# irmakguzey/SPWGNN

Measured on AMD Instinct MI355X. Metric: towers/sec fwd+bwd, 6-block batch=65k, 1/2/4/8 MI355X; achieved HBM GB/s, higher is better.
Workload: dtype f32; 1 GPU; train step fwd+BCE+bwd+Adam, 6-block towers fully connected, 65536 towers/GPU, 5 MP steps, dropout 0.1, x6 math; towers_per_gpu=65536, global_batch=65536, n_global_nodes=393216, nodes_per_tower=6, nodes_per_gpu=393216, edges_per_gpu=1966080, mp_steps=5, math=x6, parallelism=dp1

## Files before the change

include/spwgnn.h:

```cpp
#ifndef SPWGNN_H
#define SPWGNN_H

#include <stddef.h>
#include <stdint.h>

#ifdef __cplusplus
extern "C" {
#endif

#define SPWGNN_ABI_VERSION 6

#define SPWGNN_OK 0
#define SPWGNN_E_ARG (-1)
#define SPWGNN_E_SHAPE (-2)
#define SPWGNN_E_RELATION (-3)
#define SPWGNN_E_WORKSPACE (-4)
#define SPWGNN_E_CAPACITY (-5)
#define SPWGNN_E_NOTRAIN (-6)

typedef void* spwgnn_stream_t;

typedef struct spwgnn_param_info {
    const char* name;
    int64_t offset;
    int32_t rows;
    int32_t cols;
} spwgnn_param_info;

int32_t spwgnn_version(void);
int32_t spwgnn_struct_size(int32_t which);
const char* spwgnn_strerror(int32_t status);
int32_t spwgnn_param_tensor_count(void);
int64_t spwgnn_param_count(void);
// ... 80 lines not shown
#define SPWGNN_MATH_F32 0
#define SPWGNN_MATH_X6 1
#define SPWGNN_MATH_BF16 2

#define SPWGNN_K_NONE 0
#define SPWGNN_K_EDGE_FWD 1
#define SPWGNN_K_NODE_FWD 2
#define SPWGNN_K_EDGE_BWD 3
#define SPWGNN_K_NODE_BWD 4
#define SPWGNN_K_ENC_EDGE 5
#define SPWGNN_K_ENC_EDGE_BWD 6
#define SPWGNN_K_WGRAD_W2 7
#define SPWGNN_K_DA 8
#define SPWGNN_K_WGRAD_WS 9
#define SPWGNN_K_ENC_NODE 10
#define SPWGNN_K_ENC_NODE_BWD 11

int64_t spwgnn_workspace_bytes(int32_t n_nodes, int32_t n_eblocks, int32_t mp_steps, int32_t training);

int32_t spwgnn_fused_path(const spwgnn_batch* batch, const spwgnn_run* run);

int32_t spwgnn_team_max_blocks(int32_t set);

int32_t spwgnn_forward(const float* params, const spwgnn_batch* batch, const spwgnn_run* run,
                       void* workspace, int64_t workspace_bytes, float* logits,
                       spwgnn_stream_t stream);

int32_t spwgnn_backward(const float* params, const spwgnn_batch* batch, const spwgnn_run* run,
                        void* workspace, int64_t workspace_bytes, const float* dlogits,
                        float* grads, float* dprop, spwgnn_stream_t stream);

int64_t spwgnn_bce_scratch_bytes(int64_t n);
int32_t spwgnn_bce(const float* logits, const float* targets, int64_t n, float* out3,
                   float* dlogits, void* scratch, spwgnn_stream_t stream);
int32_t spwgnn_bce_accumulate(const float* logits, const float* targets, int64_t n, float* out3,
                              float* dlogits, void* scratch, const double* weights3, double* total3,
                              spwgnn_stream_t stream);
int32_t spwgnn_bce_backward(const float* params, const spwgnn_batch* batch, const spwgnn_run* run,
                            void* workspace, int64_t workspace_bytes, const float* logits,
                            const float* targets, int64_t n, float* out3, float* dlogits, void* bce_scratch,
                            const double* weights3, double* total3, float* grads, float* dprop,
                            spwgnn_stream_t stream);

int32_t spwgnn_adam(float* params, const float* grads, float* m, float* v, int64_t n, int32_t step,
                    float lr, float beta1, float beta2, float eps, float l2, float grad_scale,
                    spwgnn_stream_t stream);
// ... 31 lines not shown
```

spwgnn_amd/_lib.py:

```python
from __future__ import annotations

import ctypes as C
import os
from pathlib import Path
from typing import Optional

_LIB_PATH = Path(__file__).resolve().parent / "libspwgnn_hip.so"
_lib: Optional[C.CDLL] = None


class SpwgnnError(RuntimeError):
    pass


class ParamInfo(C.Structure):
    _fields_ = [("name", C.c_char_p), ("offset", C.c_int64), ("rows", C.c_int32), ("cols", C.c_int32)]


class PlanSizes(C.Structure):
    _fields_ = [("n_wtiles", C.c_int32), ("n_eblocks", C.c_int32), ("nw_max", C.c_int32)]


class BatchC(C.Structure):
    _fields_ = [
# ... 1 lines not shown
        ("nw_max", C.c_int32), ("flags", C.c_int32),
        ("pos", C.c_void_p), ("prop", C.c_void_p), ("node_tower", C.c_void_p), ("node_local", C.c_void_p),
        ("wtile", C.c_void_p), ("edge_src", C.c_void_p), ("edge_dst", C.c_void_p), ("blk_csr", C.c_void_p),
    ]


class PrologueC(C.Structure):
    _fields_ = [("copy_src", C.c_void_p), ("copy_dst", C.c_void_p), ("copy_bytes", C.c_int64),
                ("key", C.c_void_p), ("step", C.c_void_p), ("mode", C.c_int32), ("rank", C.c_int32),
                ("seed", C.c_uint64)]


class RunC(C.Structure):
    _fields_ = [("mp_steps", C.c_int32), ("training", C.c_int32), ("dropout", C.c_float), ("math", C.c_int32),
                ("seed", C.c_uint64), ("prof_kernel", C.c_int32), ("prof_count", C.c_int32),
                ("prof_events", C.c_void_p), ("seed_dev", C.c_void_p), ("prologue", C.c_void_p),
                ("grads_early_event", C.c_void_p)]


K_EDGE_FWD, K_NODE_FWD, K_EDGE_BWD, K_NODE_BWD, K_ENC_EDGE, K_ENC_EDGE_BWD, K_WGRAD_W2, K_DA = 1, 2, 3, 4, 5, 6, 7, 8
K_WGRAD_WS, K_ENC_NODE, K_ENC_NODE_BWD = 9, 10, 11
MATH_F32, MATH_X6, MATH_BF16 = 0, 1, 2
STEP_KEY_COUNTER, STEP_KEY_SPLITMIX = 0, 1
ABI_VERSION = 6
BATCH_RECV_BLOCKS = 1
READOUT_SUM_PROB, READOUT_MEAN_PROB, READOUT_SUM_LOGIT, READOUT_MEAN_LOGIT = 0, 1, 2, 3


def _declare(lib: C.CDLL) -> None:
    i32, i64, vp, f32 = C.c_int32, C.c_int64, C.c_void_p, C.c_float
    sig = {
        "spwgnn_version": (i32, []),
        "spwgnn_struct_size": (i32, [i32]),
        "spwgnn_strerror": (C.c_char_p, [i32]),
        "spwgnn_param_tensor_count": (i32, []),
        "spwgnn_param_count": (i64, []),
        "spwgnn_param_real_count": (i64, []),
        "spwgnn_param_tensor": (i32, [i32, C.POINTER(ParamInfo)]),
        "spwgnn_dense_to_edges": (i32, [vp, vp, i32, i32, vp, vp, vp, i64, C.POINTER(i64), vp]),
        "spwgnn_plan_size": (i32, [i32, vp, vp, i32, C.POINTER(PlanSizes)]),
        "spwgnn_plan_fill": (i32, [i32, vp, vp, vp, vp, i32, C.POINTER(PlanSizes), vp, vp, vp, vp, vp]),
        "spwgnn_plan_size_cap": (i32, [i32, vp, vp, i32, C.POINTER(PlanSizes)]),
        "spwgnn_plan_order": (i32, [i32, vp, vp, i32, vp]),
        "spwgnn_plan_fill_cap": (i32, [i32, vp, vp, vp, vp, vp, i32, C.POINTER(PlanSizes), vp, vp, vp, vp, vp]),
        "spwgnn_plan_size_recv": (i32, [i32, vp, i32, C.POINTER(PlanSizes)]),
        "spwgnn_plan_fill_recv": (i32, [i32, vp, vp, vp, vp, i32, C.POINTER(PlanSizes), vp, vp, vp, vp, vp]),
        "spwgnn_workspace_bytes": (i64, [i32, i32, i32, i32]),
        "spwgnn_fused_path": (i32, [C.POINTER(BatchC), C.POINTER(RunC)]),
        "spwgnn_team_max_blocks": (i32, [i32]),
        "spwgnn_host_device_ptr": (i32, [vp, C.POINTER(vp)]),
        "spwgnn_forward": (i32, [vp, C.POINTER(BatchC), C.POINTER(RunC), vp, i64, vp, vp]),
        "spwgnn_backward": (i32, [vp, C.POINTER(BatchC), C.POINTER(RunC), vp, i64, vp, vp, vp, vp]),
        "spwgnn_bce_scratch_bytes": (i64, [i64]),
        "spwgnn_bce": (i32, [vp, vp, i64, vp, vp, vp, vp]),
        "spwgnn_bce_accumulate": (i32, [vp, vp, i64, vp, vp, vp, vp, vp, vp]),
        "spwgnn_bce_backward": (i32, [vp, vp, vp, vp, i64, vp, vp, i64, vp, vp, vp, vp, vp, vp, vp, vp]),
        "spwgnn_adam": (i32, [vp, vp, vp, vp, i64, i32, f32, f32, f32, f32, f32, f32, vp]),
        "spwgnn_adam_dev": (i32, [vp, vp, vp, vp, i64, vp, vp, i32, f32, f32, f32, f32, f32, vp]),
        "spwgnn_adam_lr_table": (i32, [f32, f32, f32, i32, vp]),
        "spwgnn_step_advance": (i32, [vp, vp, i32, C.c_uint64, i32, vp]),
        "spwgnn_sigmoid": (i32, [vp, vp, i64, vp]),
        "spwgnn_copy_in": (i32, [vp, vp, i64, vp]),
        "spwgnn_accumulate_out3": (i32, [vp, vp, vp, vp]),
        "spwgnn_tower_readout": (i32, [vp, vp, i32, i32, vp, vp]),
    }
    for name, (res, args) in sig.items():
        fn = getattr(lib, name)
        fn.restype = res
        fn.argtypes = args


def lib() -> C.CDLL:
# ... 55 lines not shown
```

spwgnn_amd/csrc/api.hip:

```cpp
#include <cmath>
#include <cstring>
#include <cstdlib>
#include "kernels.h"
#include <vector>
#include "../../include/spwgnn.h"
static_assert(SPWGNN_MATH_F32 == spw::MATH_F32 && SPWGNN_MATH_X6 == spw::MATH_X6 && SPWGNN_MATH_BF16 == spw::MATH_BF16,
              "math ids");

namespace spw {

static inline int64_t up(int64_t x, int64_t a) { return (x + a - 1) / a * a; }

struct Ws {
    int64_t total = 0;
    int S, training;
    int64_t RN, RE, NB;
    int64_t pk;
    int64_t cw;
    int64_t zo1, co, P, a, o1, U, V, H2s;
    int64_t A, z1, z2, z3, cr;
    int64_t ed;
    int64_t mask1, mask2, zmask;
    int64_t dx, do1, g, G3, dU, dV, dP, dco, dzo2, dzo1;
    int64_t dA, dz4, dz3, dz2, dz1;
// ... 228 lines not shown
    hipStream_t st;
    mutable int k = 0;
    hipError_t before(int kid) const {
        if (r->prof_kernel != kid || !r->prof_events || k >= r->prof_count) return hipSuccess;
        return hipEventRecord(static_cast<hipEvent_t>(r->prof_events[2 * k]), st);
    }
    hipError_t after(int kid) const {
        if (r->prof_kernel != kid || !r->prof_events || k >= r->prof_count) return hipSuccess;
        hipError_t e = hipEventRecord(static_cast<hipEvent_t>(r->prof_events[2 * k + 1]), st);
        ++k;
        return e;
    }
};

#define SPW_CHECK(x)                                  \
    do {                                              \
        hipError_t e_ = (x);                          \
        if (e_ != hipSuccess) return (int32_t)e_;     \
    } while (0)

static bool rebuild_dA(const spwgnn_run* r, const spwgnn_batch* b) {
    const int m = kmath(r, kX6EdgeBwd);
    return b->nw_max <= 16 && m != MATH_F32 && !(m == MATH_X6 && !team_blocks(b->n_wtiles) && getenv_flag("SPWGNN_DA_RMW"));
}

static bool store_b16(const spwgnn_run* r, const spwgnn_batch* b) {
    return r->training && r->math == MATH_BF16 && kmath(r, kX6EncEdge) == MATH_BF16 &&
           kmath(r, kX6EncEdgeBwd) == MATH_BF16 && kmath(r, kX6Wgrad) == MATH_BF16 && rebuild_dA(r, b) &&
           !getenv_flag("SPWGNN_WG_OLD");
}

static bool store_b16_node(const spwgnn_run* r, const spwgnn_batch* b) {
    return store_b16(r, b) && kmath(r, kX6EdgeFwd) == MATH_BF16 && kmath(r, kX6NodeFwd) == MATH_BF16 &&
           kmath(r, kX6NodeBwd) == MATH_BF16 && kmath(r, kX6EdgeBwd) == MATH_BF16 && b->nw_max <= 16 &&
           !team_blocks(b->n_wtiles) && !team_blocks((b->n_nodes + 31) / 32) && !getenv_flag("SPWGNN_NODE_F32");
}

static int uv_storage(const spwgnn_run* r, const spwgnn_batch* b) {
    if (!r->training || r->math != MATH_BF16) return kUvF32;
    return store_b16_node(r, b) ? kUvB16 : kUvRound;
}

static bool fwd_fused_taken(const spwgnn_run* r, const spwgnn_batch* b) {
    const bool one_math = r->math == kmath(r, kX6EncEdge) && r->math == kmath(r, kX6EdgeFwd) &&
                          r->math == kmath(r, kX6NodeFwd);
    return one_math && fwd_fused_team(b->n_wtiles, b->nw_max, b->n_eblocks, b->n_nodes, r->math) &&
// ... 426 lines not shown
    if (!wsb || n < 2 || first < 0 || first + n > wsb->n || getenv_flag("SPWGNN_WS_NOGROUP")) return;
    const WsJob& j0 = wsb->j[first];
    const int w0 = (first + 1 < wsb->n ? wsb->j[first + 1].wg0 : wsb->wgs) - j0.wg0;
    if (w0 <= 0 || w0 % 8) return;
    for (int i = 1; i < n; ++i) {
        const WsJob& ji = wsb->j[first + i];
        const int wi = (first + i + 1 < wsb->n ? wsb->j[first + i + 1].wg0 : wsb->wgs) - ji.wg0;
        if (wi != w0 || ji.a.stages_per_wg != j0.a.stages_per_wg || ji.a.nbs != j0.a.nbs || ji.a.S != j0.a.S) return;
    }
    for (int i = 0; i < n; ++i) {
        wsb->j[first + i].gn = n;
        wsb->j[first + i].gi = i;
    }
}

int32_t run_backward(const float* params, const spwgnn_batch* b, const spwgnn_run* r, const Ws& w, char* base,
                     const float* dlogits, float* grads, float* dprop, hipStream_t st, const BceArgs* bce = nullptr) {
    (void)params;
    Ctx c{w, base};
    const int S = r->mp_steps;
    const bool rebuild = rebuild_dA(r, b);
    const bool b16 = store_b16(r, b);
    const bool n16 = store_b16_node(r, b);
    const int64_t nN = b->n_nodes;
    const float scale = (r->dropout > 0.f) ? 1.0f / (1.0f - r->dropout) : 1.0f;
    const bool zero_prop = b->prop == nullptr, need_dP0 = dprop != nullptr;
    const bool ws_skip0 = zero_prop && kmath(r, kX6Wgrad) != MATH_F32 && !getenv_flag("SPWGNN_WG_OLD");
    const bool skip_eb0 = rebuild && ws_skip0 && !need_dP0 && !team_blocks(b->n_wtiles);
    Prof prof{r, st};

    auto node_args = [&](int s) {
        const bool first = (s == S - 1);
        NodeBwdArgs nb{};
        nb.n_nodes = b->n_nodes;
        nb.first = first;
        nb.tail = 0;
        nb.dPin = first ? nullptr : c.f(w.dP_at(s + 1));
        nb.dU = first ? nullptr : c.f(w.dU_at(s + 1));
        nb.dV = first ? nullptr : c.f(w.dV_at(s + 1));
        nb.Pn = c.f(w.P_at(s + 1));
        nb.o1 = c.f(w.o1_at(s));
        nb.a = c.f(w.a_at(s));
        nb.dlogits = dlogits;
        nb.dx = c.f(w.dx_at(s));
        nb.do1 = c.f(w.do1_at(s));
        nb.g = c.f(w.g_at(s));
// ... 29 lines not shown
        return nb;
    };
    auto edge_args = [&](int s) {
        EdgeBwdArgs eb{};
        eb.n_wtiles = b->n_wtiles;
        eb.nw_max = b->nw_max;
        eb.wpg = b->nw_max <= 16 ? 4 : edge_wpg(edge_bwd_lds_per_wave(b->nw_max));
        eb.dA_accumulate = s != S - 1;
        eb.no_dA = rebuild;
        eb.wtile = b->wtile;
        eb.esrc = b->edge_src;
        eb.edst = b->edge_dst;
        eb.csr = reinterpret_cast<const uint32_t*>(b->blk_csr);
        eb.mask1 = c.u(w.m1_at(s));
        eb.mask2 = c.u(w.m2_at(s));
        eb.dh2_out = nullptr;
        eb.G3 = c.f(w.G3_at(s));
        eb.w2t = c.pk(PK_W2T);
        eb.x_w2t = r->math != MATH_F32 ? c.x6(X6_W2T) : nullptr;
        eb.dA = c.f(w.dA);
        eb.dU = c.f(w.dU_at(s));
        eb.dV = c.f(w.dV_at(s));
        eb.n16 = n16;
        return eb;
    };
    NodeBwdArgs tl{};
    if (dprop) {
        tl.n_nodes = b->n_nodes;
        tl.first = 0;
        tl.tail = 1;
        tl.dPin = c.f(w.dP_at(0));
        tl.dU = c.f(w.dU_at(0));
        tl.dV = c.f(w.dV_at(0));
        tl.dprop = dprop;
        tl.w1bt = c.pk(PK_W1BT);
        tl.w1ct = c.pk(PK_W1CT);
        if (r->math != MATH_F32) {
            tl.x_w1bt = c.x6(X6_W1BT);
            tl.x_w1ct = c.x6(X6_W1CT);
            tl.xh_w1bt = c.x6(X6_W1BT_H);
            tl.xh_w1ct = c.x6(X6_W1CT_H);
        }
        tl.n16 = n16;
    }
    DaArgs da{};
    if (rebuild) {
        da.n_eblocks = b->n_eblocks;
        da.S = S;
        da.g3_step = w.G3_at(1) - w.G3_at(0);
        da.m1_step = w.m1_at(1) - w.m1_at(0);
        da.m2_step = w.m2_at(1) - w.m2_at(0);
        da.edst = b->edge_dst;
        da.mask1 = c.u(w.mask1);
        da.mask2 = c.u(w.mask2);
        da.G3 = c.f(w.G3);
        da.dA = c.f(w.dA);
        da.x_w2t = c.x6(X6_W2T);
        da.b16 = b16;
    }
    EncEdgeBwdArgs eeb{};
    eeb.n_eblocks = b->n_eblocks;
    eeb.b16 = b16;
    eeb.dA = c.f(w.dA);
    eeb.zmask = c.u(w.zmask);
    eeb.w1at = c.pk(PK_W1AT);
    eeb.rm3t = c.pk(PK_RM3T);
    eeb.rm2t = c.pk(PK_RM2T);
    eeb.rm1t = c.pk(PK_RM1T);
    if (r->math != MATH_F32) {
        eeb.x_w1at = c.x6(X6_W1AT);
        eeb.x_rm3t = c.x6(X6_RM3T);
        eeb.x_rm2t = c.x6(X6_RM2T);
        eeb.x_rm1t = c.x6(X6_RM1T);
    }
    eeb.dz4 = c.f(w.dz4);
    eeb.dz3 = c.f(w.dz3);
    eeb.dz2 = c.f(w.dz2);
    eeb.dz1 = c.f(w.dz1);
    eeb.scale = scale;
    EncNodeBwdArgs enb{};
    enb.n_nodes = b->n_nodes;
// ... 309 lines not shown
int32_t spwgnn_fused_path(const spwgnn_batch* batch, const spwgnn_run* run) {
    const int32_t stt = validate(batch, run);
    if (stt) return stt;
    return (fwd_fused_taken(run, batch) ? 1 : 0) | (run->training && bwd_fused_taken(run, batch) ? 2 : 0);
}

int32_t spwgnn_host_device_ptr(const void* host, void** dev) {
    if (!host || !dev) return SPWGNN_E_ARG;
    void* p = nullptr;
    const hipError_t e = hipHostGetDevicePointer(&p, const_cast<void*>(host), 0);
    if (e != hipSuccess) {
        (void)hipGetLastError();
        return (int32_t)e;
    }
    if (!p) return SPWGNN_E_ARG;
    *dev = p;
    return SPWGNN_OK;
}

int32_t spwgnn_team_max_blocks(int32_t set) {
    return team_max_blocks(set);
}

int32_t spwgnn_forward(const float* params, const spwgnn_batch* batch, const spwgnn_run* run, void* workspace,
                       int64_t workspace_bytes, float* logits, spwgnn_stream_t stream) {
    int32_t stt = validate(batch, run);
    if (stt) return stt;
    if (!params || !workspace || !logits) return SPWGNN_E_ARG;
    Ws w = make_ws(batch->n_nodes, batch->n_eblocks, run->mp_steps, run->training ? 1 : 0);
    if (workspace_bytes < w.total) return SPWGNN_E_WORKSPACE;
    return run_forward(params, batch, run, w, static_cast<char*>(workspace), logits,
                       static_cast<hipStream_t>(stream));
}

int32_t spwgnn_backward(const float* params, const spwgnn_batch* batch, const spwgnn_run* run, void* workspace,
                        int64_t workspace_bytes, const float* dlogits, float* grads, float* dprop,
                        spwgnn_stream_t stream) {
    int32_t stt = validate(batch, run);
    if (stt) return stt;
    if (!run->training) return SPWGNN_E_NOTRAIN;
    if (!params || !workspace || !dlogits || !grads) return SPWGNN_E_ARG;
    Ws w = make_ws(batch->n_nodes, batch->n_eblocks, run->mp_steps, 1);
    if (workspace_bytes < w.total) return SPWGNN_E_WORKSPACE;
    return run_backward(params, batch, run, w, static_cast<char*>(workspace), dlogits, grads, dprop,
                        static_cast<hipStream_t>(stream));
}
// ... 152 lines not shown
```

spwgnn_amd/csrc/kernels.h:

```cpp
#pragma once

#ifndef SPWGNN_ONEHOT_BPERM
#define SPWGNN_ONEHOT_BPERM 1
#endif
#include "gemm_blocks.h"

namespace spw {

struct PackDesc {
    int64_t dst_off;
    int64_t src_off;
    int32_t rows, cols;
    int32_t src_rows, src_cols;
    int32_t src_ld, src_row0;
    int32_t transpose, perm;
    int32_t k4;
    int32_t bias_row;
    int64_t bias_off;
};
struct PrologueArgs {
    const uint4* src;
    uint4* dst;
    int64_t n16;
    uint64_t* key;
// ... 142 lines not shown
    int dco_sum;
    const float *w1bt, *w1ct, *wo2t, *wo1ct, *wo1at, *wo1pt, *w3t;
    const uint4 *x_w1bt, *x_w1ct, *x_wo2t, *x_wo1ct, *x_wo1at, *x_wo1pt, *x_w3t;
    const uint4 *xh_w1bt, *xh_w1ct, *xh_wo2t, *xh_wo1ct, *xh_wo1at, *xh_wo1pt;
    int n16;
    const float *bce_logits, *bce_targets;
    float* bce_dlogits;
    int64_t bce_n;
    int no_dP;
};

struct EdgeBwdArgs {
    int n_wtiles, nw_max, wpg;
    int dA_accumulate;
    int no_dA;
    const int32_t *wtile, *esrc, *edst;
    const uint32_t* csr;
    const uint32_t *mask1, *mask2;
    const float *G3, *w2t;
    float *dA, *dU, *dV;
    float* dh2_out;
    const uint4* x_w2t;
    int n16;
};

struct DaArgs {
    int n_eblocks, S;
    int b16;
    int64_t g3_step, m1_step, m2_step;
    const int32_t* edst;
    const uint32_t *mask1, *mask2;
    const float* G3;
    float* dA;
    const uint4* x_w2t;
};

struct EncEdgeBwdArgs {
    int n_eblocks;
    int b16;
    const float* dA;
    const uint32_t* zmask;
    const float *w1at, *rm3t, *rm2t, *rm1t;
    const uint4 *x_w1at, *x_rm3t, *x_rm2t, *x_rm1t;
    float *dz4, *dz3, *dz2, *dz1;
    float scale;
};

struct EncNodeBwdArgs {
    int n_nodes;
    float* dco;
    const float *co, *zo1, *om1t;
    const float* pos;
    const float *w_om0, *b_om0;
    const float* wo1ct;
    const float* do1;
    int64_t do1_step;
    int S;
// ... 146 lines not shown
    float* slab;
    int64_t nblk, blk_per_wg, count;
};
struct Pos3Batch {
    Pos3Args e, n;
    int ce, cn;
    int b16e;
};
hipError_t launch_wgrad_pos3(const Pos3Batch& p, hipStream_t st);
hipError_t launch_bce(const BceArgs& a, hipStream_t st);
hipError_t launch_adam(const AdamArgs& a, hipStream_t st);
hipError_t launch_step_advance(uint64_t* key, int32_t* step, int mode, uint64_t seed, int32_t rank, hipStream_t st);
hipError_t launch_sigmoid(const float* z, float* p, int64_t n, hipStream_t st);
hipError_t launch_accumulate_out3(const float* out3, const double* w, double* tot, hipStream_t st);
hipError_t launch_copy_in(const void* src, void* dst, int64_t n16, hipStream_t st);
hipError_t launch_tower_readout(const float* z, const int32_t* off, int n_towers, int mode, float* out, hipStream_t st);

#ifndef SPWGNN_TEAM_MAX_BLOCKS
#define SPWGNN_TEAM_MAX_BLOCKS 512
#endif
constexpr int kTeamMaxBlocks = SPWGNN_TEAM_MAX_BLOCKS;
bool team_blocks(int n_blocks);
int team_max_blocks(int set);
hipError_t launch_enc_node_team(const EncNodeArgs& a, int math, hipStream_t st);
hipError_t launch_edge_fwd_team(const EdgeFwdArgs& a, int math, hipStream_t st);
hipError_t launch_edge_bwd_team(const EdgeBwdArgs& a, int math, hipStream_t st);
hipError_t launch_dA_team(const DaArgs& a, int math, hipStream_t st);
hipError_t launch_enc_node_bwd_team(const EncNodeBwdArgs& a, int math, hipStream_t st);
hipError_t launch_node_fwd_team(const NodeFwdArgs& a, int math, hipStream_t st);
hipError_t launch_node_bwd_team(const NodeBwdArgs& a, int math, hipStream_t st);
hipError_t launch_enc_edge_team(const EncEdgeArgs& a, int math, bool train, hipStream_t st);
bool enc_pair_team(int n_eblocks, int n_nodes, int math);
hipError_t launch_enc_pair_team(const EncEdgeArgs& e, const EncNodeArgs& n, int math, bool train, hipStream_t st);
hipError_t launch_enc_edge_bwd_team(const EncEdgeBwdArgs& a, int math, hipStream_t st);
struct FwdFusedArgs {
    EncEdgeArgs ee;
    EncNodeArgs en;
    EdgeFwdArgs ef;
    NodeFwdArgs nf;
    int S, training;
    int encoders;
    int64_t rowsN, rowsE;
    int64_t m1_step, m2_step;
    float* logits;
};
bool fwd_fused_team(int n_wtiles, int nw_max, int n_eblocks, int n_nodes, int math);
// ... 27 lines not shown
```

spwgnn_amd/csrc/kernels_bwd.hip:

```cpp
#include "kernels.h"
#include <cstdlib>

namespace spw {

__global__ __launch_bounds__(256, 2) __attribute__((amdgpu_waves_per_eu(2, 2))) void k_node_bwd(NodeBwdArgs a) {
    const int lane = threadIdx.x & 63, h = lane >> 5, j = lane & 31;
    const int nb = blockIdx.x * 4 + (threadIdx.x >> 6);
    if (nb * 32 >= a.n_nodes) return;
    const int n = nb * 32 + j;
    const bool valid = n < a.n_nodes;
    const int64_t bN = (int64_t)nb * kCmBlkN, bE = (int64_t)nb * kCmBlk;
    const int pj = (h * 32 + j) * 4;

    f32x16 D[4];
    if (a.first) {
        zero_tiles(D);
    } else {
        load_cm<4>(a.dPin + bN, D, lane);
        tgemm_stream_acc<4, kKhE, kLdN, 64>(a.dU + bE + pj, D, a.w1bt, lane);
        tgemm_stream_acc<4, kKhE, kLdN, 64>(a.dV + bE + pj, D, a.w1ct, lane);
    }
    if (a.tail) {
        if (valid) {
#pragma unroll
// ... 635 lines not shown
    return hipGetLastError();
}
#ifndef SPWGNN_EBWD_PF
#define SPWGNN_EBWD_PF 2
#endif
#ifndef SPWGNN_EBWD_PF_B16
#define SPWGNN_EBWD_PF_B16 5
#endif
#ifndef SPWGNN_DA_PF_B16
#define SPWGNN_DA_PF_B16 5
#endif
#ifndef SPWGNN_DA_INTERLEAVE
#define SPWGNN_DA_INTERLEAVE 1
#endif
#ifndef SPWGNN_DA_LOCKSTEP
#define SPWGNN_DA_LOCKSTEP 1
#endif
#ifndef SPWGNN_OH_KB
#define SPWGNN_OH_KB 5
#endif
#ifndef SPWGNN_DA_DBG
#define SPWGNN_DA_DBG 0
#endif
template <bool ACCUM, bool NODA = false, int NP = 3, int DBG = 0, bool N16 = false>
__global__ __launch_bounds__(512, 1) __attribute__((amdgpu_waves_per_eu(2, 2))) void k_edge_bwd_x6(EdgeBwdArgs a) {
    constexpr int PF = NP == 1 ? SPWGNN_EBWD_PF_B16 : SPWGNN_EBWD_PF, kWaves = 8;
    __shared__ uint4 wl[50 * 3 * 64];
    for (int idx = threadIdx.x; idx < 50 * 3 * 64; idx += blockDim.x) wl[idx] = a.x_w2t[idx];
    __syncthreads();
    const int lane = threadIdx.x & 63, h = lane >> 5, i = lane & 31;
    const int wave = __builtin_amdgcn_readfirstlane(threadIdx.x >> 6);
    const int4* wtiles = reinterpret_cast<const int4*>(a.wtile);
    const int wstep = gridDim.x * kWaves;
    const WlBases wlb(wl + lane);
    struct Pre { int d, s; uint32_t w[5]; };
    auto load_pre = [&](int blk) {
        Pre p;
        const int64_t e = (int64_t)blk * 32 + i;
        p.d = a.edst[e];
        p.s = a.esrc[e];
        load_m2(a.mask2 + (int64_t)blk * kM2Blk, i, p.w);
        return p;
    };
    auto g_of = [&](int d, int n0) {
        return reinterpret_cast<const float4*>(a.G3 + cm_index<kKhE>(DBG == 3 ? n0 : (d >= 0 ? d : n0), 0) + h * 128);
    };
    struct KB { float4 g[2]; };
    auto ld = [&](const float4* G4, int kb, KB& r) {
// ... 85 lines not shown
            }
            bf16x8 ap[3];
            ap[0] = as_bf16x8(make_uint4(hw[0], hw[1], hw[2], hw[3]));
            ap[1] = as_bf16x8(make_uint4(mw[0], mw[1], mw[2], mw[3]));
            ap[2] = as_bf16x8(make_uint4(lw[0], lw[1], lw[2], lw[3]));
#pragma unroll
            for (int T = 0; T < 5; ++T) {
                const int u = (kb * 5 + T) * 3 * 64;
                bf16x8 bp[3];
                bp[0] = as_bf16x8(wlb.at(u));
                bp[1] = as_bf16x8(wlb.at(u + 64));
                bp[2] = as_bf16x8(wlb.at(u + 128));
                acc[T] = mfma32_x6<NP>(ap, bp, acc[T]);
            }
            __builtin_amdgcn_sched_barrier(0);
        }
#pragma unroll
        for (int t = 0; t < 5; ++t) {
            const uint32_t mh = m1w[t] >> (4 * h);
#pragma unroll
            for (int r = 0; r < 16; ++r) acc[t][r] = mask_bit(acc[t][r], mh, rho(r, 0));
        }
        float* dArow = a.dA + (int64_t)blk * 32 * kLdE + i;
#if SPWGNN_ONEHOT_BPERM && SPWGNN_OH_KB >= 10
        build_oh();
#endif
#pragma unroll
        for (int s = 0; s < 2; ++s) {
            uint32_t oh[4];
#pragma unroll
            for (int m = 0; m < 4; ++m) {
#if SPWGNN_ONEHOT_BPERM
                oh[m] = oh2[s][m];
#else
                uint32_t wv = 0u;
#pragma unroll
                for (int q = 0; q < 2; ++q) {
                    const int e = 2 * m + q;
                    const int d0 = __builtin_amdgcn_readlane(d, rho(8 * s + e, 0));
                    const int d1 = __builtin_amdgcn_readlane(d, rho(8 * s + e, 1));
                    const int s0 = __builtin_amdgcn_readlane(s_, rho(8 * s + e, 0));
                    const int s1 = __builtin_amdgcn_readlane(s_, rho(8 * s + e, 1));
                    const int node = i < 16 ? (h ? d1 : d0) : (h ? s1 : s0);
                    wv |= (node == key ? 0x3F80u : 0u) << (16 * q);
                }
                oh[m] = wv;
#endif
            }
            const bf16x8 ao = as_bf16x8(make_uint4(oh[0], oh[1], oh[2], oh[3]));
#pragma unroll
            for (int t = 0; t < 5; ++t) {
                uint32_t hw[4], mw[4], lw[4];
#pragma unroll
                for (int m = 0; m < 4; ++m) split2(acc[t][8 * s + 2 * m], acc[t][8 * s + 2 * m + 1], hw[m], mw[m], lw[m]);
                if constexpr (NP == 3) {
                    nacc[t] = __builtin_amdgcn_mfma_f32_32x32x16_bf16(ao, as_bf16x8(make_uint4(lw[0], lw[1], lw[2], lw[3])), nacc[t], 0, 0, 0);
                    nacc[t] = __builtin_amdgcn_mfma_f32_32x32x16_bf16(ao, as_bf16x8(make_uint4(mw[0], mw[1], mw[2], mw[3])), nacc[t], 0, 0, 0);
                }
                nacc[t] = __builtin_amdgcn_mfma_f32_32x32x16_bf16(ao, as_bf16x8(make_uint4(hw[0], hw[1], hw[2], hw[3])), nacc[t], 0, 0, 0);
#pragma unroll
                for (int r = 8 * s; r < 8 * s + 8; ++r) {
                    float* p = dArow + rho(r, h) * kLdE + 32 * t;
                    if constexpr (NODA) {
                    } else if (ACCUM) *p += acc[t][r];
                    else *p = acc[t][r];
                }
            }
        }
        cur = nxt;
        G4 = NG4;
    }
#pragma unroll
    for (int r = 0; r < 16; ++r) {
        const int row = rho(r, h);
        const int node = row & 15;
        if (node < nn) {
            float* o = row < 16 ? a.dV : a.dU;
#pragma unroll
            for (int t = 0; t < 5; ++t)
                if (32 * t + i < 2 * kKhE) {
                    if constexpr (N16) store_b16(o, cm_index<kKhE>(n0 + node, 32 * t + i), nacc[t][r]);
                    else o[cm_index<kKhE>(n0 + node, 32 * t + i)] = nacc[t][r];
                }
        }
    }
    info = ninfo;
    }
}

hipError_t launch_edge_bwd(const EdgeBwdArgs& a, int math, hipStream_t st) {
    if (math != MATH_F32 && a.nw_max <= 16 && a.no_dA && team_blocks(a.n_wtiles))
        return a.n16 ? hipErrorInvalidValue : launch_edge_bwd_team(a, math, st);
    if (a.n16 && (math != MATH_BF16 || a.nw_max > 16 || !a.no_dA)) return hipErrorInvalidValue;
    if (math != MATH_F32 && a.nw_max <= 16) {
        const dim3 g(edge_grid(a.n_wtiles, 8)), b(512);
        if (a.no_dA) {
#ifdef SPWGNN_DIAG
            static const int edbg = getenv("SPWGNN_EBWD_DBG") ? atoi(getenv("SPWGNN_EBWD_DBG")) : 0;
            if (math == MATH_BF16 && edbg == 3) {
                hipLaunchKernelGGL((k_edge_bwd_x6<false, true, 1, 3>), g, b, 0, st, a);
                return hipGetLastError();
            }
#endif
            if (math == MATH_BF16 && a.n16) hipLaunchKernelGGL((k_edge_bwd_x6<false, true, 1, 0, true>), g, b, 0, st, a);
            else if (math == MATH_BF16) hipLaunchKernelGGL((k_edge_bwd_x6<false, true, 1>), g, b, 0, st, a);
            else hipLaunchKernelGGL((k_edge_bwd_x6<false, true>), g, b, 0, st, a);
            return hipGetLastError();
        }
#ifdef SPWGNN_DIAG
        if (math != MATH_X6) return hipErrorInvalidValue;
        if (a.dA_accumulate) hipLaunchKernelGGL((k_edge_bwd_x6<true>), g, b, 0, st, a);
        else hipLaunchKernelGGL((k_edge_bwd_x6<false>), g, b, 0, st, a);
        return hipGetLastError();
#else
        return hipErrorInvalidValue;
#endif
    }
    if (a.nw_max <= 16) {
        if (a.dA_accumulate)
            hipLaunchKernelGGL((k_edge_bwd<true, true>), dim3(edge_grid(a.n_wtiles)), dim3(64 * kEdgeWaves), 0, st, a);
        else
            hipLaunchKernelGGL((k_edge_bwd<true, false>), dim3(edge_grid(a.n_wtiles)), dim3(64 * kEdgeWaves), 0, st, a);
    } else {
        const size_t lds = edge_bwd_lds_per_wave(a.nw_max) * a.wpg;
        const dim3 g((a.n_wtiles + a.wpg - 1) / a.wpg), b(64 * a.wpg);
        if (math == MATH_BF16) {
            if (a.dA_accumulate) hipLaunchKernelGGL((k_edge_bwd<false, true, true>), g, b, lds, st, a);
            else hipLaunchKernelGGL((k_edge_bwd<false, false, true>), g, b, lds, st, a);
        } else if (a.dA_accumulate) {
            hipLaunchKernelGGL((k_edge_bwd<false, true>), g, b, lds, st, a);
        } else {
            hipLaunchKernelGGL((k_edge_bwd<false, false>), g, b, lds, st, a);
        }
    }
    return hipGetLastError();
}

template <int NP = 3, bool B16 = false>
__global__ __launch_bounds__(512, 1) __attribute__((amdgpu_waves_per_eu(2, 2))) void k_dA_x6(DaArgs a) {
    constexpr int kWaves = 8, PF = NP == 1 ? SPWGNN_DA_PF_B16 : 2;
    static_assert(10 % PF == 0, "ring slots carry over between (block, step) pairs");
    __shared__ uint4 wl[50 * 3 * 64];
    for (int idx = threadIdx.x; idx < 50 * 3 * 64; idx += blockDim.x) wl[idx] = a.x_w2t[idx];
    __syncthreads();
    const int lane = threadIdx.x & 63, h = lane >> 5, i = lane & 31;
    const int wave = __builtin_amdgcn_readfirstlane(threadIdx.x >> 6);
    const WlBases wlb(wl + lane);
#if SPWGNN_DA_INTERLEAVE
    constexpr int kStride = kWaves;
    const int perw = ((a.n_eblocks + gridDim.x - 1) / gridDim.x + kWaves - 1) / kWaves * kWaves;
    const int b0 = blockIdx.x * perw + wave, b1 = min(blockIdx.x * perw + perw, a.n_eblocks);
    const int wg_b0 = blockIdx.x * perw;
    const int rounds = SPWGNN_DA_LOCKSTEP ? max(0, (b1 - wg_b0 + kWaves - 1) / kWaves) : 0;
    const int mine = SPWGNN_DA_LOCKSTEP ? max(0, (b1 - b0 + kWaves - 1) / kWaves) : 0;
#else
    constexpr int kStride = 1;
    const int nw = gridDim.x * kWaves, gw = blockIdx.x * kWaves + wave;
    const int per = (a.n_eblocks + nw - 1) / nw;
    const int b0 = gw * per, b1 = min(b0 + per, a.n_eblocks);
#endif
#if SPWGNN_DA_INTERLEAVE && SPWGNN_DA_LOCKSTEP
    auto tail_barriers = [&](int done) {
// ... 10 lines not shown
    auto load_pair = [&](int blk, int s, int d) {
        Pair p;
        const bool valid = d >= 0;
        p.G4 = reinterpret_cast<const float4*>(a.G3 + s * a.g3_step + cm_index<kKhE>(valid && SPWGNN_DA_DBG == 0 ? d : 0, 0) + h * 128);
        const uint32_t* m1 = a.mask1 + s * a.m1_step + (int64_t)blk * kLdE + i;
        if (SPWGNN_DA_DBG >= 2) {
#pragma unroll
            for (int t = 0; t < 5; ++t) p.w[t] = p.m1w[t] = valid ? 0x5a5a5a5au ^ (uint32_t)(blk * 5 + t) : 0u;
            return p;
        }
        load_m2(a.mask2 + s * a.m2_step + (int64_t)blk * kM2Blk, i, p.w);
#pragma unroll
        for (int t = 0; t < 5; ++t) {
            p.w[t] = valid ? p.w[t] : 0u;
            p.m1w[t] = m1[32 * t];
        }
        return p;
    };
    struct KB { float4 g[2]; };
    auto ld = [&](const float4* G4, int kb, KB& r) {
#pragma unroll
        for (int c = 0; c < 2; ++c) r.g[c] = G4[64 * min(2 * kb + c, kKhE / 4 - 1)];
    };
    int blk = b0, s = a.S - 1;
    int d = a.edst[(int64_t)blk * 32 + i];
    Pair cur = load_pair(blk, s, d);
    KB ring[PF];
#pragma unroll
    for (int k = 0; k < PF; ++k) ld(cur.G4, k, ring[k]);
    f32x16 dacc[5];
    zero_tiles(dacc);
    for (;;) {
        const bool last_step = s == 0;
        const bool has_next = !last_step || blk + kStride < b1;
        const int nblk = last_step ? (blk + kStride < b1 ? blk + kStride : blk) : blk;
        const int ns = last_step ? a.S - 1 : s - 1;
        const int nd = last_step ? a.edst[(int64_t)nblk * 32 + i] : d;
        const Pair nxt = load_pair(nblk, max(ns, 0), nd);
        const uint64_t mlo = h == 0 ? ((uint64_t)cur.w[1] << 32 | cur.w[0])
                                    : ((uint64_t)cur.w[4] << 52 | (uint64_t)cur.w[3] << 20 | (cur.w[2] >> 12));
        const uint32_t mhi = h == 0 ? (cur.w[2] & 0xfffu) : (cur.w[4] >> 12);
        f32x16 acc[5];
        zero_tiles(acc);
#pragma unroll
        for (int kb = 0; kb < 10; ++kb) {
            KB& cr = ring[kb % PF];
            float xv[8];
#pragma unroll
            for (int c = 0; c < 2; ++c) {
                const int q = 2 * kb + c;
                const uint32_t bits = q < 16 ? (uint32_t)(mlo >> (4 * q)) : (q < 19 ? mhi >> (4 * q - 64) : 0u);
                xv[4 * c + 0] = mask_bit(cr.g[c].x, bits, 0);
                xv[4 * c + 1] = mask_bit(cr.g[c].y, bits, 1);
                xv[4 * c + 2] = mask_bit(cr.g[c].z, bits, 2);
                xv[4 * c + 3] = mask_bit(cr.g[c].w, bits, 3);
            }
            uint32_t hw[4], mw[4], lw[4];
#pragma unroll
            for (int m = 0; m < 4; ++m) split2(xv[2 * m], xv[2 * m + 1], hw[m], mw[m], lw[m]);
// ... 35 lines not shown
                float* dArow = a.dA + (int64_t)blk * 32 * kLdE + i;
#pragma unroll
                for (int t = 0; t < 5; ++t)
#pragma unroll
                    for (int r = 0; r < 16; ++r) dArow[rho(r, h) * kLdE + 32 * t] = dacc[t][r];
            }
            zero_tiles(dacc);
#if SPWGNN_DA_INTERLEAVE && SPWGNN_DA_LOCKSTEP
            __syncthreads();
#endif
        }
        if (!has_next) break;
        blk = nblk;
        s = ns;
        d = nd;
        cur = nxt;
    }
#if SPWGNN_DA_INTERLEAVE && SPWGNN_DA_LOCKSTEP
    tail_barriers(mine);
#endif
}

hipError_t launch_dA(const DaArgs& a, int math, hipStream_t st) {
    if ((math == MATH_X6 || math == MATH_BF16) && team_blocks(a.n_eblocks)) return launch_dA_team(a, math, st);
    const dim3 g(edge_grid(a.n_eblocks, 8)), b(512);
    if (math == MATH_BF16 && a.b16) hipLaunchKernelGGL((k_dA_x6<1, true>), g, b, 0, st, a);
    else if (math == MATH_BF16) hipLaunchKernelGGL((k_dA_x6<1>), g, b, 0, st, a);
    else hipLaunchKernelGGL((k_dA_x6<3>), g, b, 0, st, a);
    return hipGetLastError();
}
hipError_t launch_enc_edge_bwd(const EncEdgeBwdArgs& a, int math, hipStream_t st) {
    constexpr int NC = 1, NW = 4, NWB = SPWGNN_ENC_NW_B16;
    if ((math == MATH_X6 || math == MATH_BF16) && team_blocks(a.n_eblocks)) return launch_enc_edge_bwd_team(a, math, st);
    const dim3 g((a.n_eblocks + 4 * NC - 1) / (4 * NC)), gb((a.n_eblocks + NWB * NC - 1) / (NWB * NC));
    if (math == MATH_BF16) {
        if (a.b16) hipLaunchKernelGGL((k_enc_edge_bwd_x6<NC, 1, true, NWB>), gb, dim3(64 * NWB), 0, st, a);
        else hipLaunchKernelGGL((k_enc_edge_bwd_x6<NC, 1, false, NW>), g, dim3(256), 0, st, a);
        return hipGetLastError();
    }
    if (math == MATH_X6) {
        constexpr int NWX = SPWGNN_ENC_NW_X6;
        const dim3 gx((a.n_eblocks + NWX * NC - 1) / (NWX * NC));
        hipLaunchKernelGGL((k_enc_edge_bwd_x6<NC, 3, false, NWX>), gx, dim3(64 * NWX), 0, st, a);
        return hipGetLastError();
    }
    hipLaunchKernelGGL(k_enc_edge_bwd, dim3((a.n_eblocks + 3) / 4), dim3(256), 0, st, a);
    return hipGetLastError();
}
template <int NP, int NW = 0>
__global__ __launch_bounds__(256, 2) void k_enc_node_bwd_x6(EncNodeBwdArgs a) {
    const int lane = threadIdx.x & 63, h = lane >> 5, j = lane & 31;
// ... 59 lines not shown
```

spwgnn_amd/engine.py:

```python
from __future__ import annotations

import ctypes as C
import os
import weakref
from dataclasses import dataclass
from typing import Optional

import torch

from . import _lib, params as P
from .batch import TowerBatch

REF_MP_STEPS = 5
REF_DROPOUT = 0.1


def _stream(device: torch.device) -> int:
    return torch.cuda.current_stream(device).cuda_stream


def _require_gpu(t: torch.Tensor, what: str):
    if t.device.type != "cuda":
        raise _lib.SpwgnnError(f"{what} must be a HIP device tensor (got {t.device}); the HIP path has no CPU fallback")

# ... 119 lines not shown


def fused_path(batch: TowerBatch, run: RunConfig) -> int:
    b = batch.cstruct()
    r = run.cstruct()
    st = _lib.lib().spwgnn_fused_path(C.byref(b), C.byref(r))
    if st < 0:
        _lib.check(st, "spwgnn_fused_path")
    return int(st)


def team_max_blocks(set_to: Optional[int] = None) -> int:
    return int(_lib.lib().spwgnn_team_max_blocks(-1 if set_to is None else int(set_to)))


class wide_kernels:

    def __enter__(self):
        self._prev = team_max_blocks(0)
        return self

    def __exit__(self, *exc):
        team_max_blocks(self._prev)
        return False


def forward(flat_params: torch.Tensor, batch: TowerBatch, run: RunConfig, ws: Workspace,
            logits: Optional[torch.Tensor] = None) -> torch.Tensor:
    _require_gpu(flat_params, "params")
    if flat_params.dtype != torch.float32 or not flat_params.is_contiguous() or flat_params.numel() != P.flat_size():
        raise ValueError("params must be a contiguous fp32 flat buffer of spwgnn_param_count() floats")
    nbytes = workspace_bytes(batch, run)
    buf = ws.get(nbytes)
    if logits is None:
        logits = _poison(torch.empty(batch.n_nodes, dtype=torch.float32, device=batch.device))
    b = batch.cstruct()
    r = run.cstruct(with_prologue=True)
    st = _lib.lib().spwgnn_forward(flat_params.data_ptr(), C.byref(b), C.byref(r), buf.data_ptr(), buf.numel(),
                                   logits.data_ptr(), _stream(batch.device))
    ws.fwd_key = Workspace.key(batch, run) if st == 0 else None
    ws.fwd_batch = weakref.ref(batch) if st == 0 else None
    _lib.check(st, "spwgnn_forward")
    return logits


def backward(flat_params: torch.Tensor, batch: TowerBatch, run: RunConfig, ws: Workspace, dlogits: torch.Tensor,
# ... 147 lines not shown
```

Baseline: 2.692 million towers/s.

## Store per-step dh1pre tiles in workspace slabs to skip dA rebuild steps

The x6 edge-backward kernel now writes its per-step pre-activation gradient tiles into spare dz workspace slabs for the last few message-passing steps. The dA kernel then sums those stored tiles directly instead of recomputing them, and runs its rebuild loop only over the remaining steps. This trades recomputation in the dA kernel for extra nontemporal HBM writes and reads. It applies only on the non-team, non-fused x6 path, and only when the slab geometry fits.

Result: faster. 2.744 million towers/s (median of 6 runs) (+1.9%).

```diff
diff --git a/include/spwgnn.h b/include/spwgnn.h
--- a/include/spwgnn.h
+++ b/include/spwgnn.h
@@ -8,7 +8,7 @@
 extern "C" {
 #endif
 
-#define SPWGNN_ABI_VERSION 6
+#define SPWGNN_ABI_VERSION 7
 
 #define SPWGNN_OK 0
 #define SPWGNN_E_ARG (-1)
@@ -135,6 +135,8 @@
 
 int32_t spwgnn_team_max_blocks(int32_t set);
 
+int32_t spwgnn_da_stored_steps(int32_t set);
+
 int32_t spwgnn_forward(const float* params, const spwgnn_batch* batch, const spwgnn_run* run,
                        void* workspace, int64_t workspace_bytes, float* logits,
                        spwgnn_stream_t stream);
diff --git a/spwgnn_amd/_lib.py b/spwgnn_amd/_lib.py
--- a/spwgnn_amd/_lib.py
+++ b/spwgnn_amd/_lib.py
@@ -47,7 +47,7 @@
 K_WGRAD_WS, K_ENC_NODE, K_ENC_NODE_BWD = 9, 10, 11
 MATH_F32, MATH_X6, MATH_BF16 = 0, 1, 2
 STEP_KEY_COUNTER, STEP_KEY_SPLITMIX = 0, 1
-ABI_VERSION = 6
+ABI_VERSION = 7
 BATCH_RECV_BLOCKS = 1
 READOUT_SUM_PROB, READOUT_MEAN_PROB, READOUT_SUM_LOGIT, READOUT_MEAN_LOGIT = 0, 1, 2, 3
 
@@ -73,6 +73,7 @@
         "spwgnn_workspace_bytes": (i64, [i32, i32, i32, i32]),
         "spwgnn_fused_path": (i32, [C.POINTER(BatchC), C.POINTER(RunC)]),
         "spwgnn_team_max_blocks": (i32, [i32]),
+        "spwgnn_da_stored_steps": (i32, [i32]),
         "spwgnn_host_device_ptr": (i32, [vp, C.POINTER(vp)]),
         "spwgnn_forward": (i32, [vp, C.POINTER(BatchC), C.POINTER(RunC), vp, i64, vp, vp]),
         "spwgnn_backward": (i32, [vp, C.POINTER(BatchC), C.POINTER(RunC), vp, i64, vp, vp, vp, vp]),
diff --git a/spwgnn_amd/csrc/api.hip b/spwgnn_amd/csrc/api.hip
--- a/spwgnn_amd/csrc/api.hip
+++ b/spwgnn_amd/csrc/api.hip
@@ -1,3 +1,5 @@
+#include <algorithm>
+#include <atomic>
 #include <cmath>
 #include <cstring>
 #include <cstdlib>
@@ -274,6 +276,23 @@
 static bool rebuild_dA(const spwgnn_run* r, const spwgnn_batch* b) {
     const int m = kmath(r, kX6EdgeBwd);
     return b->nw_max <= 16 && m != MATH_F32 && !(m == MATH_X6 && !team_blocks(b->n_wtiles) && getenv_flag("SPWGNN_DA_RMW"));
+}
+
+#ifndef SPWGNN_DA_STORED
+#define SPWGNN_DA_STORED 3
+#endif
+static std::atomic<int> g_da_stored{SPWGNN_DA_STORED};
+int da_stored_steps(int set) {
+    return set >= 0 ? g_da_stored.exchange(set) : g_da_stored.load(std::memory_order_relaxed);
+}
+static bool bwd_fused_taken(const spwgnn_run* r, const spwgnn_batch* b);
+static int da_stored_planned(const spwgnn_run* r, const spwgnn_batch* b, const Ws& w) {
+    if (!rebuild_dA(r, b) || kmath(r, kX6EdgeBwd) != MATH_X6 || team_blocks(b->n_wtiles) || team_blocks(b->n_eblocks) ||
+        bwd_fused_taken(r, b))
+        return 0;
+    const int64_t step = w.dz3 - w.dz4;
+    if (step < (int64_t)b->n_eblocks * kCmBlk || w.dz2 - w.dz3 != step || w.dz1 - w.dz2 != step) return 0;
+    return std::max(0, std::min({da_stored_steps(-1), 4, r->mp_steps - 1}));
 }
 
 static bool store_b16(const spwgnn_run* r, const spwgnn_batch* b) {
@@ -746,6 +765,8 @@
     const bool rebuild = rebuild_dA(r, b);
     const bool b16 = store_b16(r, b);
     const bool n16 = store_b16_node(r, b);
+    const int n_stored = da_stored_planned(r, b, w);
+    const int64_t slab_step = w.dz3 - w.dz4;
     const int64_t nN = b->n_nodes;
     const float scale = (r->dropout > 0.f) ? 1.0f / (1.0f - r->dropout) : 1.0f;
     const bool zero_prop = b->prop == nullptr, need_dP0 = dprop != nullptr;
@@ -821,6 +842,7 @@
         eb.dU = c.f(w.dU_at(s));
         eb.dV = c.f(w.dV_at(s));
         eb.n16 = n16;
+        eb.dh1_slab = S - 1 - s < n_stored ? c.f(w.dz4) + (S - 1 - s) * slab_step : nullptr;
         return eb;
     };
     NodeBwdArgs tl{};
@@ -856,6 +878,9 @@
         da.dA = c.f(w.dA);
         da.x_w2t = c.x6(X6_W2T);
         da.b16 = b16;
+        da.n_stored = n_stored;
+        da.slab_step = slab_step;
+        da.slab = n_stored ? c.f(w.dz4) : nullptr;
     }
     EncEdgeBwdArgs eeb{};
     eeb.n_eblocks = b->n_eblocks;
@@ -1211,6 +1236,10 @@
     return team_max_blocks(set);
 }
 
+int32_t spwgnn_da_stored_steps(int32_t set) {
+    return da_stored_steps(set);
+}
+
 int32_t spwgnn_forward(const float* params, const spwgnn_batch* batch, const spwgnn_run* run, void* workspace,
                        int64_t workspace_bytes, float* logits, spwgnn_stream_t stream) {
     int32_t stt = validate(batch, run);
diff --git a/spwgnn_amd/csrc/kernels.h b/spwgnn_amd/csrc/kernels.h
--- a/spwgnn_amd/csrc/kernels.h
+++ b/spwgnn_amd/csrc/kernels.h
@@ -188,6 +188,7 @@
     float* dh2_out;
     const uint4* x_w2t;
     int n16;
+    float* dh1_slab;
 };
 
 struct DaArgs {
@@ -199,6 +200,9 @@
     const float* G3;
     float* dA;
     const uint4* x_w2t;
+    int n_stored;
+    int64_t slab_step;
+    const float* slab;
 };
 
 struct EncEdgeBwdArgs {
@@ -391,6 +395,7 @@
 constexpr int kTeamMaxBlocks = SPWGNN_TEAM_MAX_BLOCKS;
 bool team_blocks(int n_blocks);
 int team_max_blocks(int set);
+int da_stored_steps(int set);
 hipError_t launch_enc_node_team(const EncNodeArgs& a, int math, hipStream_t st);
 hipError_t launch_edge_fwd_team(const EdgeFwdArgs& a, int math, hipStream_t st);
 hipError_t launch_edge_bwd_team(const EdgeBwdArgs& a, int math, hipStream_t st);
diff --git a/spwgnn_amd/csrc/kernels_bwd.hip b/spwgnn_amd/csrc/kernels_bwd.hip
--- a/spwgnn_amd/csrc/kernels_bwd.hip
+++ b/spwgnn_amd/csrc/kernels_bwd.hip
@@ -681,8 +681,30 @@
 #ifndef SPWGNN_DA_DBG
 #define SPWGNN_DA_DBG 0
 #endif
-template <bool ACCUM, bool NODA = false, int NP = 3, int DBG = 0, bool N16 = false>
+constexpr int kSlabT4 = (2 * kKhE - 128), kSlabT4Base = 4 * 4 * 64;
+static_assert(kSlabT4Base + 8 * kSlabT4 == kCmBlk / 4, "a stored dh1pre block fills a chunk-major block exactly");
+#ifndef SPWGNN_SLAB_NT
+#define SPWGNN_SLAB_NT 1
+#endif
+typedef float slab_f4 __attribute__((ext_vector_type(4)));
+__device__ __forceinline__ void slab_store(float4* p, const float4& v) {
+#if SPWGNN_SLAB_NT
+    __builtin_nontemporal_store(slab_f4{v.x, v.y, v.z, v.w}, reinterpret_cast<slab_f4*>(p));
+#else
+    *p = v;
+#endif
+}
+__device__ __forceinline__ float4 slab_load(const float4* p) {
+#if SPWGNN_SLAB_NT
+    const slab_f4 v = __builtin_nontemporal_load(reinterpret_cast<const slab_f4*>(p));
+    return make_float4(v.x, v.y, v.z, v.w);
+#else
+    return *p;
+#endif
+}
+template <bool ACCUM, bool NODA = false, int NP = 3, int DBG = 0, bool N16 = false, bool SLAB = false>
 __global__ __launch_bounds__(512, 1) __attribute__((amdgpu_waves_per_eu(2, 2))) void k_edge_bwd_x6(EdgeBwdArgs a) {
+    static_assert(!SLAB || (NODA && NP == 3 && !N16), "stored dh1pre steps: the x6 rebuild form only");
     constexpr int PF = NP == 1 ? SPWGNN_EBWD_PF_B16 : SPWGNN_EBWD_PF, kWaves = 8;
     __shared__ uint4 wl[50 * 3 * 64];
     for (int idx = threadIdx.x; idx < 50 * 3 * 64; idx += blockDim.x) wl[idx] = a.x_w2t[idx];
@@ -814,6 +836,7 @@
             for (int r = 0; r < 16; ++r) acc[t][r] = mask_bit(acc[t][r], mh, rho(r, 0));
         }
         float* dArow = a.dA + (int64_t)blk * 32 * kLdE + i;
+        float4* slab4 = SLAB ? reinterpret_cast<float4*>(a.dh1_slab) + (int64_t)blk * (kCmBlk / 4) : nullptr;
 #if SPWGNN_ONEHOT_BPERM && SPWGNN_OH_KB >= 10
         build_oh();
 #endif
@@ -857,6 +880,14 @@
                     } else if (ACCUM) *p += acc[t][r];
                     else *p = acc[t][r];
                 }
+                if constexpr (SLAB) {
+#pragma unroll
+                    for (int q = 2 * s; q < 2 * s + 2; ++q) {
+                        const float4 v = make_float4(acc[t][4 * q], acc[t][4 * q + 1], acc[t][4 * q + 2], acc[t][4 * q + 3]);
+                        if (t < 4) slab_store(slab4 + (4 * t + q) * 64 + lane, v);
+                        else if (i < kSlabT4) slab_store(slab4 + kSlabT4Base + (q * 2 + h) * kSlabT4 + i, v);
+                    }
+                }
             }
         }
         cur = nxt;
@@ -881,6 +912,7 @@
 }
 
 hipError_t launch_edge_bwd(const EdgeBwdArgs& a, int math, hipStream_t st) {
+    if (a.dh1_slab && (math != MATH_X6 || a.nw_max > 16 || !a.no_dA || team_blocks(a.n_wtiles))) return hipErrorInvalidValue;
     if (math != MATH_F32 && a.nw_max <= 16 && a.no_dA && team_blocks(a.n_wtiles))
         return a.n16 ? hipErrorInvalidValue : launch_edge_bwd_team(a, math, st);
     if (a.n16 && (math != MATH_BF16 || a.nw_max > 16 || !a.no_dA)) return hipErrorInvalidValue;
@@ -896,6 +928,7 @@
 #endif
             if (math == MATH_BF16 && a.n16) hipLaunchKernelGGL((k_edge_bwd_x6<false, true, 1, 0, true>), g, b, 0, st, a);
             else if (math == MATH_BF16) hipLaunchKernelGGL((k_edge_bwd_x6<false, true, 1>), g, b, 0, st, a);
+            else if (a.dh1_slab) hipLaunchKernelGGL((k_edge_bwd_x6<false, true, 3, 0, false, true>), g, b, 0, st, a);
             else hipLaunchKernelGGL((k_edge_bwd_x6<false, true>), g, b, 0, st, a);
             return hipGetLastError();
         }
@@ -928,8 +961,9 @@
     return hipGetLastError();
 }
 
-template <int NP = 3, bool B16 = false>
+template <int NP = 3, bool B16 = false, bool SLAB = false>
 __global__ __launch_bounds__(512, 1) __attribute__((amdgpu_waves_per_eu(2, 2))) void k_dA_x6(DaArgs a) {
+    static_assert(!SLAB || (NP == 3 && !B16), "stored dh1pre steps: x6 only");
     constexpr int kWaves = 8, PF = NP == 1 ? SPWGNN_DA_PF_B16 : 2;
     static_assert(10 % PF == 0, "ring slots carry over between (block, step) pairs");
     __shared__ uint4 wl[50 * 3 * 64];
@@ -986,7 +1020,8 @@
 #pragma unroll
         for (int c = 0; c < 2; ++c) r.g[c] = G4[64 * min(2 * kb + c, kKhE / 4 - 1)];
     };
-    int blk = b0, s = a.S - 1;
+    const int s_top = SLAB ? a.S - 1 - a.n_stored : a.S - 1;
+    int blk = b0, s = s_top;
     int d = a.edst[(int64_t)blk * 32 + i];
     Pair cur = load_pair(blk, s, d);
     KB ring[PF];
@@ -994,11 +1029,41 @@
     for (int k = 0; k < PF; ++k) ld(cur.G4, k, ring[k]);
     f32x16 dacc[5];
     zero_tiles(dacc);
+    auto slab_sum = [&](int sblk) {
+        const float4* sp = reinterpret_cast<const float4*>(a.slab) + (int64_t)sblk * (kCmBlk / 4);
+        for (int k = 0; k < a.n_stored; ++k, sp += a.slab_step / 4) {
+            auto part = [&](auto T0c, auto T1c) {
+                constexpr int T0 = decltype(T0c)::value, T1 = decltype(T1c)::value;
+                float4 v[T1 - T0][4];
+#pragma unroll
+                for (int t = T0; t < T1; ++t)
+#pragma unroll
+                    for (int q = 0; q < 4; ++q) {
+                        if (t < 4) v[t - T0][q] = slab_load(sp + (4 * t + q) * 64 + lane);
+                        else v[t - T0][q] = i < kSlabT4 ? slab_load(sp + kSlabT4Base + (q * 2 + h) * kSlabT4 + i) : make_float4(0.f, 0.f, 0.f, 0.f);
+                    }
+#pragma unroll
+                for (int t = T0; t < T1; ++t)
+#pragma unroll
+                    for (int q = 0; q < 4; ++q) {
+                        dacc[t][4 * q + 0] += v[t - T0][q].x;
+                        dacc[t][4 * q + 1] += v[t - T0][q].y;
+                        dacc[t][4 * q + 2] += v[t - T0][q].z;
+                        dacc[t][4 * q + 3] += v[t - T0][q].w;
+                    }
+            };
+            part(std::integral_constant<int, 0>{}, std::integral_constant<int, 3>{});
+            part(std::integral_constant<int, 3>{}, std::integral_constant<int, 5>{});
+        }
+    };
     for (;;) {
+        if constexpr (SLAB) {
+            if (s == s_top) slab_sum(blk);
+        }
         const bool last_step = s == 0;
         const bool has_next = !last_step || blk + kStride < b1;
         const int nblk = last_step ? (blk + kStride < b1 ? blk + kStride : blk) : blk;
-        const int ns = last_step ? a.S - 1 : s - 1;
+        const int ns = last_step ? s_top : s - 1;
         const int nd = last_step ? a.edst[(int64_t)nblk * 32 + i] : d;
         const Pair nxt = load_pair(nblk, max(ns, 0), nd);
         const uint64_t mlo = h == 0 ? ((uint64_t)cur.w[1] << 32 | cur.w[0])
@@ -1080,11 +1145,15 @@
 }
 
 hipError_t launch_dA(const DaArgs& a, int math, hipStream_t st) {
+    if (a.n_stored > 0 && (math != MATH_X6 || team_blocks(a.n_eblocks))) return hipErrorInvalidValue;
     if ((math == MATH_X6 || math == MATH_BF16) && team_blocks(a.n_eblocks)) return launch_dA_team(a, math, st);
     const dim3 g(edge_grid(a.n_eblocks, 8)), b(512);
     if (math == MATH_BF16 && a.b16) hipLaunchKernelGGL((k_dA_x6<1, true>), g, b, 0, st, a);
     else if (math == MATH_BF16) hipLaunchKernelGGL((k_dA_x6<1>), g, b, 0, st, a);
-    else hipLaunchKernelGGL((k_dA_x6<3>), g, b, 0, st, a);
+    else if (a.n_stored > 0) {
+        if (a.n_stored >= a.S || !a.slab || a.b16) return hipErrorInvalidValue;
+        hipLaunchKernelGGL((k_dA_x6<3, false, true>), g, b, 0, st, a);
+    } else hipLaunchKernelGGL((k_dA_x6<3>), g, b, 0, st, a);
     return hipGetLastError();
 }
 hipError_t launch_enc_edge_bwd(const EncEdgeBwdArgs& a, int math, hipStream_t st) {
diff --git a/spwgnn_amd/engine.py b/spwgnn_amd/engine.py
--- a/spwgnn_amd/engine.py
+++ b/spwgnn_amd/engine.py
@@ -165,6 +165,27 @@
 
     def __exit__(self, *exc):
         team_max_blocks(self._prev)
+        return False
+
+
+DA_STORED_DEFAULT = 3
+
+
+def da_stored_steps(set_to: Optional[int] = None) -> int:
+    return int(_lib.lib().spwgnn_da_stored_steps(-1 if set_to is None else int(set_to)))
+
+
+class da_stored:
+
+    def __init__(self, k: int):
+        self._k = int(k)
+
+    def __enter__(self):
+        self._prev = da_stored_steps(self._k)
+        return self
+
+    def __exit__(self, *exc):
+        da_stored_steps(self._prev)
         return False
 
 
```
